# Khrylx/EgoPose

Measured on AMD Instinct MI355X. Metric: env-steps/sec (whole node) ego_mimic PPO, higher is better.
Workload: dtype f64 (rollout kernels K1-K6, physics state) + f32 (policy/value nets)

## Files before the change

egopose_amd/_lib.py:

```python
from __future__ import annotations

import ctypes as C
import os

HERE = os.path.dirname(os.path.abspath(__file__))
LIB_PATH = os.path.join(HERE, "libegopose_hip.so")

EGP_OK = 0
EGP_EXPERT_ROW = 168
EGP_LSTM_GATES_UNIT_MAJOR = 1

c_int_p = C.POINTER(C.c_int32)
c_dbl_p = C.POINTER(C.c_double)
vp = C.c_void_p


class ModelDesc(C.Structure):
    _fields_ = [
        ("nq", C.c_int32), ("nv", C.c_int32), ("nu", C.c_int32), ("nbody", C.c_int32), ("nM", C.c_int32),
        ("body_qpos_start", c_int_p), ("body_ndof", c_int_p), ("dof_parentid", c_int_p), ("dof_Madr", c_int_p),
        ("ee_body", c_int_p),
        ("jkp", c_dbl_p), ("jkd", c_dbl_p), ("a_ref", c_dbl_p), ("a_scale", c_dbl_p), ("torque_lim", c_dbl_p),
        ("b_diffw", c_dbl_p),
        ("sub_dt", C.c_double), ("frame_skip", C.c_int32), ("episode_len", C.c_int32),
# ... 37 lines not shown
class PolicyDesc(C.Structure):
    _fields_ = [("n", C.c_int32),
                ("ctx_rows", vp), ("ctx_row_stride", C.c_int64), ("ctx_dim", C.c_int32),
                ("t_idx", vp),
                ("state", vp), ("state_dim", C.c_int32),
                ("ctx", vp),
                ("qpos", vp), ("qvel", vp), ("phase_t", vp),
                ("zf_in", vp), ("zf_out", vp), ("clip", C.c_double),
                ("y", vp), ("y2", vp),
                ("zf_workspace", vp),
                ("layers", C.POINTER(MlpLayer)), ("n_layers", C.c_int32), ("activation", C.c_int32),
                ("log_std", vp), ("noise", vp),
                ("action", vp), ("mean_out", vp),
                ("cell", C.POINTER(MlpLayer)),
                ("h", vp), ("c", vp), ("hc_row_stride", C.c_int64),
                ("vctx_rows", vp), ("vctx_row_stride", C.c_int64), ("vctx_dim", C.c_int32),
                ("vlayers", C.POINTER(MlpLayer)), ("n_vlayers", C.c_int32), ("vactivation", C.c_int32),
                ("value_out", vp),
                ("stage_src", vp), ("stage_dst", vp), ("stage_bytes", C.c_int64)]


class LstmDesc(C.Structure):
    _fields_ = [("T", C.c_int32), ("B", C.c_int32), ("hidden", C.c_int32), ("n_problems", C.c_int32), ("reverse_mask", C.c_int32),
                ("w_hh", vp),
                ("gates_x", vp), ("ld_g", C.c_int32),
                ("h_out", vp * 4), ("ld_h", C.c_int32),
                ("gates_save", vp), ("cells_save", vp),
                ("last_only", C.c_int32),
                ("seq_base", vp),
                ("dh_out", vp * 4), ("ld_dh", C.c_int32),
                ("d_pre", vp),
                ("d_bias", vp), ("d_bias_rows", C.c_int32),
                ("seq_order", vp), ("seq_steps", vp), ("leave_skipped", C.c_int32)]


class GemmDesc(C.Structure):
    _fields_ = [("M", C.c_int32), ("N", C.c_int32), ("K", C.c_int32),
                ("A", vp), ("lda", C.c_int64), ("a_kcontig", C.c_int32),
                ("B", vp), ("ldb", C.c_int64), ("b_kcontig", C.c_int32),
                ("C", vp), ("ldc", C.c_int64),
                ("bias", vp), ("relu", C.c_int32),
                ("mask", vp), ("ldmask", C.c_int64),
                ("terms", C.c_int32), ("splits", C.c_int32), ("accumulate", C.c_int32),
                ("bias_grad", vp), ("workspace", vp),
                ("a_rows", vp), ("A2", vp), ("lda2", C.c_int64), ("a_split", C.c_int32), ("a_src_rows", C.c_int64),
                ("b_krows", vp), ("B2", vp), ("ldb2", C.c_int64), ("b_split", C.c_int32), ("b_src_rows", C.c_int64),
                ("c_rows", vp), ("a_krows", vp),
                ("act_kind", C.c_int32), ("mask_kind", C.c_int32)]


class PpoLossDesc(C.Structure):
    _fields_ = [("n", C.c_int32), ("n_pol", C.c_int32), ("act_dim", C.c_int32),
                ("rows", vp), ("pred", vp), ("returns", vp),
                ("mean", vp), ("ld_mean", C.c_int64),
                ("actions", vp), ("ld_act", C.c_int64),
                ("log_std", vp), ("adv", vp),
                ("fixed_logp", vp), ("write_fixed", C.c_int32),
                ("clip_eps", C.c_double), ("inv_n_val", C.c_double), ("inv_n_exp", C.c_double),
                ("d_pred", vp), ("d_mean", vp), ("ld_dmean", C.c_int64), ("d_log_std", vp),
                ("losses", vp), ("workspace", vp)]


class MinibatchPlanDesc(C.Structure):
    _fields_ = [("n", C.c_int32), ("state_dim", C.c_int32), ("act_dim", C.c_int32), ("batch", C.c_int32),
                ("perm", vp),
                ("states", vp), ("ld_states", C.c_int64),
# ... 142 lines not shown
    "egp_pose_features_f32": (C.c_int, [vp, vp, vp, vp, _i32, _i32, vp, vp, vp, vp, vp, vp, vp, vp]),
    "egp_zfilter_workspace_bytes": (_i64, [_i32, _i32]),
    "egp_zfilter_f64": (C.c_int, [vp, vp, _i32, _i32, vp, vp, _i32, _f64, vp, vp, vp]),
    "egp_zfilter_f32": (C.c_int, [vp, vp, _i32, _i32, vp, vp, _i32, _f64, vp, vp, vp]),
    "egp_obs_zfilter_f64": (C.c_int, [vp, vp, vp, vp, vp, _i32, vp, vp, _f64, vp, vp, _i32, vp, vp]),
    "egp_obs_zfilter_f32": (C.c_int, [vp, vp, vp, vp, vp, _i32, vp, vp, _f64, vp, vp, _i32, vp, vp]),
    "egp_gae_workspace_bytes": (_i64, [_i32]),
    "egp_gae_f64": (C.c_int, [vp, vp, vp, _i32, _f64, _f64, vp, vp, vp, vp, vp]),
    "egp_gae_f32": (C.c_int, [vp, vp, vp, _i32, _f64, _f64, vp, vp, vp, vp, vp]),
    "egp_gae_standardize_f64": (C.c_int, [vp, _i32, vp, vp]),
    "egp_gae_standardize_f32": (C.c_int, [vp, _i32, vp, vp]),
    "egp_lstm_gate_layout": (_i32, []),
    "egp_gather_concat_f32": (C.c_int, [vp, _i64, vp, vp, _i64, _i32, _i32, _i32, vp, _i64, vp]),
    "egp_scatter_rows_f32": (C.c_int, [vp, _i64, vp, _i32, _i32, vp, _i64, vp]),
    "egp_gemm_workspace_floats": (_i64, [_i32, _i32, _i32, _i32]),
    "egp_gemm_f32": (C.c_int, [C.POINTER(GemmDesc), vp]),
    "egp_ppo_loss_workspace_bytes": (_i64, [_i32, _i32, _i32]),
    "egp_ppo_loss_f32": (C.c_int, [C.POINTER(PpoLossDesc), vp]),
    "egp_ppo_stats_workspace_bytes": (_i64, [_i32, _i32, _i32]),
    "egp_ppo_stats_f32": (C.c_int, [C.POINTER(PpoStatsDesc), vp]),
    "egp_minibatch_plan_f32": (C.c_int, [C.POINTER(MinibatchPlanDesc), vp]),
    "egp_ppo_loss_mb_f32": (C.c_int, [C.POINTER(PpoLossMbDesc), vp]),
    "egp_gail_rows_f32": (C.c_int, [C.POINTER(GailRowsDesc), vp]),
    "egp_gail_rows_bwd_f32": (C.c_int, [C.POINTER(GailRowsDesc), vp]),
    "egp_bce_logits_workspace_bytes": (_i64, [_i32]),
    "egp_bce_logits_f32": (C.c_int, [C.POINTER(BceLogitsDesc), vp]),
    "egp_tcn_conv_f32": (C.c_int, [C.POINTER(TcnDesc), vp]),
    "egp_adam_workspace_bytes": (_i64, []),
    "egp_adam_step_f32": (C.c_int, [_i32, C.POINTER(AdamSegment), vp, vp, vp, vp, vp, vp, vp]),
    "egp_adam_step_f64": (C.c_int, [_i32, C.POINTER(AdamSegment), vp, vp, vp, vp, vp, vp, vp, vp]),
    "egp_adam_step_f64g": (C.c_int, [_i32, C.POINTER(AdamSegment), vp, vp, vp, vp, vp, vp, vp]),
    "egp_lstm_fwd_f32": (C.c_int, [C.POINTER(LstmDesc), vp]),
    "egp_lstm_bwd_f32": (C.c_int, [C.POINTER(LstmDesc), vp]),
    "egp_rollout_tick_pre": (C.c_int, [vp, _i32, _i32, _i32, _i32, vp, _i32, vp, vp]),
    "egp_rollout_tick_apply": (C.c_int, [vp, _i32, _i32, _i32, _i32, vp, vp]),
    "egp_obs_zfilter_split_max_rows": (C.c_int32, []),
    "egp_obs_zfilter_stats_f64": (C.c_int, [vp, vp, vp, vp, vp, _i32, vp, vp]),
    "egp_obs_zfilter_apply_f64": (C.c_int, [vp, vp, vp, vp, _i32, vp, vp, C.c_double, vp, vp, vp, vp]),
    "egp_rollout_tick_post": (C.c_int, [vp, _i32, _i32, _i32, _i32, vp, vp, vp, vp]),
    "egp_rollout_reset": (C.c_int, [vp, _i32, _i32, _i32, _i32, vp, _i32, vp, vp, vp, vp, vp, vp, vp, vp, vp]),
    "egp_engine_group_stream": (vp, [vp, _i32]),
    "egp_debug_burn": (C.c_int, [C.c_int64, _i32, vp, vp]),
    "egp_set_dynamics_model": (C.c_int, [vp, C.POINTER(DynamicsDesc)]),
    "egp_dynamics_f64": (C.c_int, [vp, vp, vp, _i32, vp, C.c_int64, vp, vp, vp]),
    "egp_set_pose2d_bodies": (C.c_int, [vp, c_int_p, c_int_p]),
    "egp_pose2d_f64": (C.c_int, [vp, vp, vp, vp, vp, vp, vp, C.c_int64, vp]),
    "egp_mlp_pack_floats": (C.c_int64, [_i32, _i32]),
    "egp_mlp_pack_f32": (C.c_int, [vp, C.c_int64, _i32, _i32, vp, vp]),
    "egp_policy_step_f32": (C.c_int, [C.POINTER(PolicyDesc), vp]),
    "egp_physics_register": (C.c_int, [C.POINTER(PhysicsVtable), _i32, C.POINTER(vp)]),
    "egp_physics_create_surrogate": (C.c_int, [C.POINTER(SurrogateDesc), _i32, C.POINTER(vp)]),
    "egp_physics_destroy": (C.c_int, [vp]),
    "egp_physics_name": (C.c_char_p, [vp]),
    "egp_physics_n_env": (_i32, [vp]),
    "egp_physics_reset_host": (C.c_int, [vp, _i32, vp, vp]),
    "egp_physics_step_host": (C.c_int, [vp, _i32, vp]),
    "egp_physics_drain_host": (C.c_int, [vp, _i32, vp, vp, vp, vp, vp]),
    "egp_engine_create": (C.c_int, [vp, vp, C.POINTER(EngineDesc), C.POINTER(vp)]),
    "egp_engine_destroy": (C.c_int, [vp]),
    "egp_engine_state": (C.c_int, [vp] + [C.POINTER(vp)] * 7),
    "egp_engine_reset": (C.c_int, [vp, vp, _i32, vp, vp, vp]),
    "egp_engine_step_async": (C.c_int, [vp, _i32, vp, vp, vp]),
    "egp_engine_wait": (C.c_int, [vp, _i32, vp]),
    "egp_engine_timing": (C.c_int, [vp, c_dbl_p, c_dbl_p, c_dbl_p, C.POINTER(_i64)]),
    "egp_engine_reset_timing": (C.c_int, [vp]),
    "egp_engine_inertia_uploads": (_i64, [vp]),
# ... 60 lines not shown
```

egopose_amd/csrc/egp_kernels.hip:

```cpp
#include <hip/hip_runtime.h>
#include <math.h>
#include <stdarg.h>
#include <stdio.h>
#include <stdlib.h>
#include <string.h>

#include <atomic>
#include <map>
#include <mutex>

#include "egp_internal.hpp"
#include "egp_dynamics_dev.hpp"
#include "egp_quat.hpp"
#include "egp_filter_dev.hpp"

namespace egp {

static thread_local char g_err[512] = "";
void set_error(const char *fmt, ...) {
    va_list ap;
    va_start(ap, fmt);
    vsnprintf(g_err, sizeof(g_err), fmt, ap);
    va_end(ap);
}
// ... 1713 lines not shown
static int dev_copy(egp_ctx *ctx, const T *host, size_t count, const T **out) {
    void *d = nullptr;
    EGP_HIP_CHECK(hipMalloc(&d, count * sizeof(T)));
    ctx->allocs.push_back(d);
    EGP_HIP_CHECK(hipMemcpy(d, host, count * sizeof(T), hipMemcpyHostToDevice));
    *out = (const T *)d;
    return EGP_OK;
}

static int fill_reward(egp_ctx *ctx, const egp_model_desc *d) {
    RewardW &w = ctx->rw;
    w.w_p = d->w_p; w.w_v = d->w_v; w.w_e = d->w_e; w.w_rp = d->w_rp; w.w_rv = d->w_rv;
    w.w_sum = d->w_p + d->w_v + d->w_e + d->w_rp + d->w_rv;
    w.k_p = d->k_p; w.k_v = d->k_v; w.k_e = d->k_e; w.k_rh = d->k_rh; w.k_rq = d->k_rq; w.k_rl = d->k_rl; w.k_ra = d->k_ra;
    w.v_ord = d->v_ord; w.decay = d->decay; w.episode_len = d->episode_len;
    EGP_REQUIRE(d->v_ord >= 1.0, "v_ord must be >= 1");
    EGP_REQUIRE(d->episode_len > 0, "episode_len must be positive");
    return EGP_OK;
}

extern "C" {

const char *egp_last_error(void) { return g_err; }
const char *egp_version(void) { return "egopose_hip 0.2.0 (gfx950)"; }
int64_t egp_abi_sizeof(const char *name) {
    if (!name) return -1;
#define EGP_ABI_SIZE(T) if (!strcmp(name, #T)) return (int64_t)sizeof(T);
    EGP_ABI_SIZE(egp_model_desc) EGP_ABI_SIZE(egp_expert_table) EGP_ABI_SIZE(egp_gemm_desc)
    EGP_ABI_SIZE(egp_dynamics_desc) EGP_ABI_SIZE(egp_mlp_layer) EGP_ABI_SIZE(egp_physics_vtable)
    EGP_ABI_SIZE(egp_surrogate_desc) EGP_ABI_SIZE(egp_engine_desc) EGP_ABI_SIZE(egp_rollout_tick)
    EGP_ABI_SIZE(egp_ppo_loss_desc) EGP_ABI_SIZE(egp_adam_segment) EGP_ABI_SIZE(egp_host_probe_result)
    EGP_ABI_SIZE(egp_minibatch_plan_desc) EGP_ABI_SIZE(egp_ppo_loss_mb_desc) EGP_ABI_SIZE(egp_tcn_desc)
    EGP_ABI_SIZE(egp_policy_desc) EGP_ABI_SIZE(egp_gail_rows_desc) EGP_ABI_SIZE(egp_bce_logits_desc)
    EGP_ABI_SIZE(egp_lstm_desc) EGP_ABI_SIZE(egp_ppo_stats_desc)
#undef EGP_ABI_SIZE
    return -1;
}
int32_t egp_obs_dim(const egp_ctx *ctx) { return ctx ? ctx->dm.obs_dim : -1; }

int egp_create(const egp_model_desc *d, int device, egp_ctx **out) {
    EGP_REQUIRE(d && out, "desc/out is NULL");
    EGP_REQUIRE(d->nv > 6 && d->nv <= EGP_MAX_NV, "nv must be in (6, 64]");
    EGP_REQUIRE(d->nq == d->nv + 1 && d->nu == d->nv - 6, "expects one free root joint + hinges (nq=nv+1, nu=nv-6)");
    EGP_REQUIRE(d->nbody >= 2 && d->nbody + 5 <= EGP_MAX_BODY, "nbody must be in [2, 27]");
    EGP_REQUIRE(d->nM > 0 && d->nM <= PD_NM_MAX, "nM out of range");
    EGP_REQUIRE(d->body_qpos_start && d->body_ndof && d->dof_parentid && d->dof_Madr && d->ee_body, "skeleton table is NULL");
    EGP_REQUIRE(d->jkp && d->jkd && d->a_ref && d->a_scale && d->torque_lim && d->b_diffw, "gain table is NULL");
    EGP_REQUIRE(d->sub_dt > 0 && d->frame_skip > 0, "timestep/frame_skip must be positive");
    EGP_REQUIRE(26 + 4 * (d->nbody - 1) <= 106 && 106 + 3 * (d->nbody - 1) <= EGP_EXPERT_ROW, "expert row overflow");
    EGP_HIP_CHECK(hipSetDevice(device));
    egp_ctx *ctx = new egp_ctx();
    ctx->device = device;
    ctx->frame_skip = d->frame_skip;
    int rc = fill_reward(ctx, d);
    if (rc != EGP_OK) { delete ctx; return rc; }
    DevModel &m = ctx->dm;
    m.nq = d->nq; m.nv = d->nv; m.nu = d->nu; m.nbody = d->nbody; m.nM = d->nM;
    m.sub_dt = d->sub_dt;
    m.dt = d->sub_dt * d->frame_skip;
    m.obs_heading = d->obs_heading != 0; m.obs_keep = d->obs_keep_root_heading != 0; m.obs_root = d->obs_coord_root != 0;
    m.obs_vel = d->obs_vel;
    m.action_torque = d->action_torque != 0;
    if (m.obs_vel < 0 || m.obs_vel > 2) { delete ctx; set_error("obs_vel must be 0 (full), 1 (root) or 2 (none)"); return EGP_E_INVALID; }
    m.obs_phase = d->obs_phase != 0;
    m.episode_len = d->episode_len;
    if (m.obs_phase && d->episode_len <= 0) { delete ctx; set_error("obs_phase needs episode_len > 0"); return EGP_E_INVALID; }
    m.obs_dim = obs_width(d->nq, d->nv, m.obs_heading, m.obs_vel, m.obs_phase);
// ... 592 lines not shown
```

egopose_amd/csrc/egp_lstm.hip:

```cpp
#include <hip/hip_runtime.h>
#include <math.h>
#include <stdlib.h>

#include "egp_internal.hpp"

namespace egp {

constexpr int KC = 64;

__device__ __forceinline__ float sigmoidf_(float x) { return __builtin_amdgcn_rcpf(1.0f + __expf(-x)); }
__device__ __forceinline__ float tanhf_(float x) { return 2.0f * __builtin_amdgcn_rcpf(1.0f + __expf(-2.0f * x)) - 1.0f; }

typedef float f32x4 __attribute__((ext_vector_type(4)));

template <typename V> __device__ __forceinline__ void st_save(V *p, V v) { __builtin_nontemporal_store(v, p); }
template <typename V> __device__ __forceinline__ V ld_save(const V *p) { return __builtin_nontemporal_load(p); }
template <typename V> __device__ __forceinline__ void st_dpre(V *p, V v) { __builtin_nontemporal_store(v, p); }

struct LstmGroup {
    int ld_g;
    int rev_mask;
    int ld_h;
    int ld_dh;
    long c_stride;
// ... 293 lines not shown
        for (int d = 0; d < PD; ++d) EGP_LSTM_FETCH(s0 - PD - d, d)
#pragma unroll
        for (int d = 0; d < PD; ++d)
            do_step(s0 - d, cg[d], cc_[d], cdh[d], d + 1 < PD ? cc_[d + 1 < PD ? d + 1 : 0] : pc[0]);
    }
#pragma unroll
    for (int d = 0; d < PD - 1; ++d)
        if (s0 - d >= 0) do_step(s0 - d, pg[d], pc[d], pdh[d], pc[d + 1]);
#undef EGP_LSTM_FETCH
    if (grp.db) {
        __syncthreads();
#pragma unroll
        for (int qq = 0; qq < NP; ++qq) {
            const int p = threadIdx.x + NT * qq;
            *reinterpret_cast<f32x4 *>(&s_d[p / LH][4 * (p % LH)]) = dsum[qq];
        }
        __syncthreads();
        if (grp.db_rows) {
            for (int p = threadIdx.x; p < ROWS * LG; p += NT) {
                const int r = p / LG, c = p % LG;
                if (FULL || r0 + r < B) grp.db[((long)prob * B + r0 + r) * LG + c] = s_d[r][c];
            }
        } else {
            for (int c = threadIdx.x; c < LG; c += NT) {
                float a = 0.f;
#pragma unroll
                for (int r = 0; r < ROWS; ++r) a += s_d[r][c];
                atomicAdd(grp.db + prob * LG + c, a);
            }
        }
    }
}

}

using namespace egp;

static int lstm_quads(int B) { return B >= 4096 ? 2 : 1; }

template <int NQ, int LH>
static void launch_fwd_mfma_t(bool full, bool train, bool last, int P, const float *gx, const float *w_hh, int T, int B, const LstmGroup &g,
                              float *gates_save, float *cells_save, hipStream_t s) {
    const dim3 grid((B + 4 * NQ - 1) / (4 * NQ), P), block(4 * LH);
    if (last && full) k_lstm_fwd_mfma<NQ, LH, true, LSTM_ST_LAST><<<grid, block, 0, s>>>(gx, w_hh, T, B, g, nullptr, nullptr);
    else if (last) k_lstm_fwd_mfma<NQ, LH, false, LSTM_ST_LAST><<<grid, block, 0, s>>>(gx, w_hh, T, B, g, nullptr, nullptr);
    else if (full && train) k_lstm_fwd_mfma<NQ, LH, true, LSTM_ST_TRAIN><<<grid, block, 0, s>>>(gx, w_hh, T, B, g, gates_save, cells_save);
    else if (full) k_lstm_fwd_mfma<NQ, LH, true, LSTM_ST_STEP><<<grid, block, 0, s>>>(gx, w_hh, T, B, g, gates_save, cells_save);
    else if (train) k_lstm_fwd_mfma<NQ, LH, false, LSTM_ST_TRAIN><<<grid, block, 0, s>>>(gx, w_hh, T, B, g, gates_save, cells_save);
    else k_lstm_fwd_mfma<NQ, LH, false, LSTM_ST_STEP><<<grid, block, 0, s>>>(gx, w_hh, T, B, g, gates_save, cells_save);
}
static void launch_fwd_mfma(int hidden, int P, const float *gx, const float *w_hh, int T, int B, const LstmGroup &g,
                            float *gates_save, float *cells_save, hipStream_t s, bool last = false) {
    const int nq = hidden == 64 ? lstm_quads(B) : 1;
    const bool full = B % (4 * nq) == 0, train = gates_save != nullptr;
    if (hidden == 128) launch_fwd_mfma_t<1, 128>(full, train, last, P, gx, w_hh, T, B, g, gates_save, cells_save, s);
    else if (nq >= 2) launch_fwd_mfma_t<2, 64>(full, train, last, P, gx, w_hh, T, B, g, gates_save, cells_save, s);
    else launch_fwd_mfma_t<1, 64>(full, train, last, P, gx, w_hh, T, B, g, gates_save, cells_save, s);
}

template <int NQ, int LH>
static void launch_bwd_mfma_t(bool full, int P, const float *gates_save, const float *cells_save, const float *w_hh, int T, int B,
                              const LstmGroup &g, float *d_pre, hipStream_t s) {
    const dim3 grid((B + 4 * NQ - 1) / (4 * NQ), P), block(4 * LH);
    if (full) k_lstm_bwd_mfma<NQ, LH, true><<<grid, block, 0, s>>>(gates_save, cells_save, w_hh, T, B, g, d_pre);
    else k_lstm_bwd_mfma<NQ, LH, false><<<grid, block, 0, s>>>(gates_save, cells_save, w_hh, T, B, g, d_pre);
}
// ... 22 lines not shown
    }
    const int ld_g = d->ld_g ? d->ld_g : 4 * H * P, ld_io = bwd ? d->ld_dh : d->ld_h;
    EGP_REQUIRE(ld_g >= 4 * H * P && ld_g % 4 == 0, "gate row stride below n_problems * 4H or not a multiple of 4");
    EGP_REQUIRE(ld_io == 0 || ld_io >= H, "h_out / dh_out row stride below the hidden size");
    EGP_REQUIRE((d->seq_order == nullptr) == (d->seq_steps == nullptr), "seq_order and seq_steps go together");
    EGP_REQUIRE((d->gates_save == nullptr) == (d->cells_save == nullptr), "gates_save and cells_save go together");
    EGP_REQUIRE(d->w_hh && (bwd ? d->gates_save && d->d_pre : d->gates_x != nullptr), "NULL pointer");
    if (!bwd) {
        EGP_REQUIRE(!d->seq_base || !d->gates_save || d->gates_save != d->gates_x,
                    "a frame table cannot double as the saved gates (rows are shared between sequences)");
        EGP_REQUIRE(!last || P == 1, "last_only sweeps one problem");
        EGP_REQUIRE(!last || !d->gates_save, "last_only saves nothing (inference)");
        EGP_REQUIRE(!last || !d->seq_order, "last_only takes no seq_order / seq_steps");
        EGP_REQUIRE(!last || d->seq_base, "last_only needs seq_base (windows of a frame table)");
    }
    LstmGroup g = {};
    g.ld_g = ld_g; g.rev_mask = d->reverse_mask; g.c_stride = (long)T * B * H;
    g.order = d->seq_order; g.steps = d->seq_steps; g.leave_skipped = d->seq_steps && d->leave_skipped;
    (bwd ? g.ld_dh : g.ld_h) = ld_io ? ld_io : H;
    for (int p = 0; p < P; ++p) {
        EGP_REQUIRE(bwd ? d->dh_out[p] != nullptr : d->h_out[p] != nullptr, "NULL h_out / dh_out of a problem");
        if (bwd) g.dh[p] = d->dh_out[p]; else g.h[p] = d->h_out[p];
    }
    if (bwd) {
        g.db = d->d_bias; g.db_rows = db_rows;
        launch_bwd_mfma(H, P, d->gates_save, d->cells_save, d->w_hh, T, B, g, d->d_pre, (hipStream_t)stream);
    } else {
        g.seq_base = d->seq_base;
        launch_fwd_mfma(H, P, d->gates_x, d->w_hh, T, B, g, d->gates_save, d->cells_save, (hipStream_t)stream, last);
    }
    return after_launch(bwd ? "k_lstm_bwd_mfma" : "k_lstm_fwd_mfma");
}

extern "C" {

int32_t egp_lstm_gate_layout(void) { return EGP_LSTM_GATES_UNIT_MAJOR; }
int egp_lstm_fwd_f32(const egp_lstm_desc *desc, void *stream) { return lstm_sweep(desc, false, stream); }
int egp_lstm_bwd_f32(const egp_lstm_desc *desc, void *stream) { return lstm_sweep(desc, true, stream); }

}
```

egopose_amd/lstm.py:

```python
from __future__ import annotations

import ctypes as C

import numpy as np
import torch

from . import _lib as L
from . import gemm as G

HIDDEN_SIZES = (64, 128)


def available(x, cell):
    return (x.is_cuda and x.dtype == torch.float32 and cell.hidden_size in HIDDEN_SIZES
            and cell.weight_hh.dtype == torch.float32 and cell.bias_ih is not None)


def _s():
    return L.current_stream()


_LAYOUT_CHECKED = False


# ... 69 lines not shown

    @staticmethod
    def backward(ctx, dh):
        lib = _lib()
        x2, w_in, w_hh, h_buf, gates, cells = ctx.saved_tensors
        T, B, D = ctx.shape
        HIDDEN = w_hh.shape[1]
        h = h_buf
        dpre = torch.empty(T, B, 4 * HIDDEN, dtype=h.dtype, device=h.device)
        dh = dh.contiguous()
        d = _desc(T, B, HIDDEN, 1, 1 if ctx.reverse else 0, w_hh, gates_save=gates, cells_save=cells,
                  dh_out=_slabs([dh.data_ptr()]), d_pre=dpre)
        L.check(lib.egp_lstm_bwd_f32(d, _s()), "egp_lstm_bwd_f32")
        h_prev = h_buf[1:] if ctx.reverse else h_buf[:T]
        _, inv = _gate_perm(HIDDEN, h.device)
        if G.enabled():
            d2 = dpre.view(T * B, 4 * HIDDEN)
            dw_ih, dbias = G.linear_wgrad(d2, x2, want_bias=True)
            dw_hh = G.linear_wgrad(d2, h_prev.reshape(T * B, HIDDEN), want_bias=False)
            dw_ih, dw_hh, dbias = dw_ih.index_select(0, inv), dw_hh.index_select(0, inv), dbias.index_select(0, inv)
            d_w_ih = dw_ih if ctx.needs_input_grad[1] else None
            d_w_hh = dw_hh if ctx.needs_input_grad[2] else None
            d_b = dbias if (ctx.needs_input_grad[3] or ctx.needs_input_grad[4]) else None
        else:
            xh1 = torch.cat((x2.view(T, B, D), h_prev, h.new_ones(T, B, 1)), 2)
            dw = torch.bmm(dpre.transpose(1, 2), xh1).sum(0).index_select(0, inv)
            d_w_ih = dw[:, :D].contiguous() if ctx.needs_input_grad[1] else None
            d_w_hh = dw[:, D:D + HIDDEN].contiguous() if ctx.needs_input_grad[2] else None
            d_b = dw[:, D + HIDDEN].contiguous() if (ctx.needs_input_grad[3] or ctx.needs_input_grad[4]) else None
        d_x = dpre.view(T * B, 4 * HIDDEN).mm(w_in).view(T, B, D) if ctx.needs_input_grad[0] else None
        return d_x, d_w_ih, d_w_hh, d_b, d_b, None, None


class LstmGroup(torch.autograd.Function):

    @staticmethod
    def forward(ctx, x, reverse_mask, P, width, train, ragged, frames, *params):
        lib = _lib()
        T, B, D = x.shape
        w_ih, w_hh, b_ih, b_hh = params[0::4], params[1::4], params[2::4], params[3::4]
        H = w_hh[0].shape[1]
        x2 = x.reshape(T * B, D)
        pord = [p for p in range(P) if not (reverse_mask >> p) & 1] + [p for p in range(P) if (reverse_mask >> p) & 1]
        nf = sum(1 for p in range(P) if not (reverse_mask >> p) & 1)
        kmask = sum(1 << q for q in range(nf, P))
        bperm, _ = _stacked_perm(H, P, x.device)
        w_in = torch.cat([w_ih[p] for p in pord], 0).index_select(0, bperm)
        bias = (torch.cat([b_ih[p] for p in pord]) + torch.cat([b_hh[p] for p in pord])).index_select(0, bperm)
        rows = None
        if ragged is not None and ragged.rows is not None and 0 < nf and G.enabled() and G.fused_rows_available() \
                and ragged.T == T and ragged.rows.shape[0] >= 4096 and D >= 32:
            rows = ragged.rows
        seq_base, gates_buf = None, None
        if frames is not None and G.enabled():
            table, seq_base = frames
            gx = G.linear_fwd(table, w_in, bias)
            gates_buf = torch.empty(T * B, P * 4 * H, dtype=x.dtype, device=x.device) if train else None
        elif rows is not None:
            gx = torch.empty(T * B, P * 4 * H, dtype=x.dtype, device=x.device)
            nfc = nf * 4 * H
            G.gemm(x2, w_in[:nfc], True, True, bias=bias[:nfc], a_rows=rows, c_rows=rows, out=gx[:, :nfc])
            if nf < P:
                G.gemm(x2, w_in[nfc:], True, True, bias=bias[nfc:], out=gx[:, nfc:])
        elif G.enabled():
            gx = G.linear_fwd(x2, w_in, bias)
        else:
            gx = torch.addmm(bias, x2, w_in.t())
        w_hh_all = torch.stack([w_hh[p].contiguous() for p in pord], 0)
        n_out, W = P // width, width * H
        h_buf = torch.empty(n_out, T + 2, B, W, dtype=x.dtype, device=x.device)
        h_buf[:, 0].zero_()
        h_buf[:, T + 1].zero_()
        cells = torch.empty(P, T, B, H, dtype=x.dtype, device=x.device) if train else None
        base, esz = h_buf.data_ptr(), h_buf.element_size()
        ptrs = _slabs([base + esz * (((p // width) * (T + 2) + 1) * B * W + (p % width) * H) for p in pord])
        order, steps = (ragged.order, ragged.steps) if ragged is not None else (None, None)
        leave = int(rows is not None and train)
        gates = gates_buf if seq_base is not None else (gx if train else None)
        d = _desc(T, B, H, P, kmask, w_hh_all, gates_x=gx, h_out=ptrs, ld_h=W, gates_save=gates, cells_save=cells, seq_base=seq_base,
                  seq_order=order, seq_steps=steps, leave_skipped=leave)
        L.check(lib.egp_lstm_fwd_f32(d, _s()), "egp_lstm_fwd_f32")
        outs = tuple(h_buf[i, 1:T + 1] for i in range(n_out))
        if train:
            ctx.save_for_backward(x2, w_in, w_hh_all, h_buf, gates, cells)
            ctx.meta = (T, B, D, H, P, width, reverse_mask)
            ctx.ragged, ctx.rows, ctx.pord, ctx.nf, ctx.kmask, ctx.leave = ragged, rows, pord, nf, kmask, leave
        return outs

    @staticmethod
    def backward(ctx, *douts):
        lib = _lib()
        x2, w_in, w_hh_all, h_buf, gates, cells = ctx.saved_tensors
        T, B, D, H, P, width, reverse_mask = ctx.meta
        W = width * H
        _, inv = _gate_perm(H, x2.device)
        douts = [d.contiguous() if d is not None else h_buf.new_zeros(T, B, W) for d in douts]
        ragged, rows, pord, nf, kmask = ctx.ragged, ctx.rows, ctx.pord, ctx.nf, ctx.kmask
        esz = h_buf.element_size()
        ptrs = _slabs([douts[p // width].data_ptr() + esz * (p % width) * H for p in pord])
        dpre = torch.empty(T * B, P * 4 * H, dtype=x2.dtype, device=x2.device)
        db_rows = torch.empty(P, B, 4 * H, dtype=x2.dtype, device=x2.device)
        order, steps = (ragged.order, ragged.steps) if ragged is not None else (None, None)
        leave = int(bool(ctx.leave) and not ctx.needs_input_grad[0])
        d = _desc(T, B, H, P, kmask, w_hh_all, gates_save=gates, cells_save=cells, dh_out=ptrs, ld_dh=W, d_pre=dpre,
                  d_bias=db_rows, d_bias_rows=1, seq_order=order, seq_steps=steps, leave_skipped=leave)
        L.check(lib.egp_lstm_bwd_f32(d, _s()), "egp_lstm_bwd_f32")
        db = db_rows.sum(1)
        d3 = dpre.view(T, B, P * 4 * H)
        use_g = G.enabled()
        nfc = nf * 4 * H
        if rows is not None:
            n_rows = rows.shape[0]
            parts = [G.gemm(dpre[:, :nfc], x2, False, False, splits=G.pick_splits(nfc, D, n_rows), a_krows=rows, b_krows=rows)]
            if nf < P:
                parts.append(G.linear_wgrad(dpre[:, nfc:], x2, want_bias=False))
            dw_ih_all = torch.cat(parts, 0)
        elif use_g:
            dw_ih_all = G.linear_wgrad(dpre, x2, want_bias=False)
        else:
            dw_ih_all = torch.bmm(d3.transpose(1, 2), x2.view(T, B, D)).sum(0)
        grads = [None] * (4 * P)
        _, binv = _stacked_perm(H, P, x2.device)
        dw_ih_t = dw_ih_all.index_select(0, binv)
        db_t = db.reshape(-1).index_select(0, binv).view(P, 4 * H)
        for q, p in enumerate(pord):
            rev = (kmask >> q) & 1
            slab = h_buf[p // width, 2:] if rev else h_buf[p // width, :T]
            h_prev = slab[:, :, (p % width) * H:(p % width + 1) * H]
            if use_g:
                dq, hq = dpre[:, q * 4 * H:(q + 1) * 4 * H], slab.reshape(T * B, W)[:, (p % width) * H:(p % width + 1) * H]
                if rows is not None and not rev:
                    dw_hh = G.gemm(dq, hq, False, False, splits=G.pick_splits(4 * H, H, rows.shape[0]), a_krows=rows, b_krows=rows).index_select(0, inv)
                else:
                    dw_hh = G.linear_wgrad(dq, hq, want_bias=False).index_select(0, inv)
            else:
                dw_hh = torch.bmm(d3[:, :, q * 4 * H:(q + 1) * 4 * H].transpose(1, 2), h_prev).sum(0).index_select(0, inv)
            dw_ih = dw_ih_t[q * 4 * H:(q + 1) * 4 * H]
            d_b = db_t[q]
            grads[4 * p:4 * p + 4] = [dw_ih, dw_hh, d_b, d_b]
        d_x = dpre.mm(w_in).view(T, B, D) if ctx.needs_input_grad[0] else None
        return (d_x, None, None, None, None, None, None, *grads)


def _wants_grad(x, params):
    return torch.is_grad_enabled() and (x.requires_grad or any(p.requires_grad for p in params))


def group_available(x, cells):
    if not cells or len(cells) > 4:
        return False
    c0 = cells[0]
    return all(available(x, c) and c.hidden_size == c0.hidden_size and c.input_size == c0.input_size for c in cells)


class Ragged:

    def __init__(self, order, steps, rows, n_seq, T):
        self.order, self.steps, self.rows, self.n_seq, self.T = order, steps, rows, n_seq, T


def ragged_order(seq_steps, device, T=None):
    st = np.asarray(torch.as_tensor(seq_steps).cpu().numpy(), dtype=np.int64).reshape(-1)
    B = st.shape[0]
    order = np.argsort(-st, kind="stable")
    st_sorted = st[order]
    rows = None
    if T is not None and B > 0:
        wg = np.maximum.reduceat(st_sorted, np.arange(0, B, 8))
        t_wg = np.minimum(np.repeat(wg, 8)[:B], int(T))
        n = int(t_wg.sum())
        if n < 0.9 * T * B:
            t_seq = np.empty(B, np.int64)
            t_seq[order] = t_wg
            stepped = np.arange(int(T), dtype=np.int64)[:, None] < t_seq[None, :]
            rows = torch.as_tensor(np.flatnonzero(stepped), dtype=torch.int64, device=device)
    return Ragged(torch.as_tensor(order, dtype=torch.int32, device=device), torch.as_tensor(st_sorted, dtype=torch.int32, device=device),
                  rows, B, T)


def lstm_group(x, cells, reverses, pairs=False, ragged=None, frames=None):
    mask = sum(1 << i for i, r in enumerate(reverses) if r)
    params = [t for c in cells for t in (c.weight_ih, c.weight_hh, c.bias_ih, c.bias_hh)]
    if ragged is not None and ragged.n_seq != x.shape[1]:
        ragged = None
    if frames is not None:
        table, base = frames
        ok = (table.is_cuda and table.dtype == x.dtype and table.dim() == 2 and table.shape[1] == x.shape[2] and table.is_contiguous()
              and base.dtype == torch.int32 and base.is_cuda and base.is_contiguous() and base.shape[0] == x.shape[1] and not x.requires_grad)
        if not ok:
            frames = None
    return list(LstmGroup.apply(x.contiguous(), mask, len(cells), 2 if pairs else 1, _wants_grad(x, params), ragged, frames, *params))


WINDOW_CALLS = 0


def window_available(table, cell):
    return available(table, cell)


@torch.no_grad()
def window_last(cell, table, seq_base, steps, reverse, out):
    global WINDOW_CALLS
    H, B = cell.hidden_size, seq_base.shape[0]
    if not (table.dim() == 2 and table.is_contiguous() and window_available(table, cell)):
        raise ValueError("window_last needs a contiguous float32 (F, D) table on the device and an LSTMCell of hidden size 64 or 128")
    if not (seq_base.is_cuda and seq_base.dtype == torch.int32 and seq_base.dim() == 1 and seq_base.is_contiguous()):
        raise ValueError("seq_base must be a contiguous int32 device vector")
    if not (out.is_cuda and out.dtype == torch.float32 and out.shape == (B, H) and (H == 1 or out.stride(1) == 1)
            and (B <= 1 or out.stride(0) >= H)):
        raise ValueError("out must be float32 (B, H) = (%d, %d) device rows, got %s" % (B, H, tuple(out.shape)))
    if steps < 1:
        raise ValueError("a window has at least one step, got %d" % steps)
    if B == 0:
        return out
    lo, hi = int(seq_base.min()), int(seq_base.max())
    if lo < 0 or hi + steps > table.shape[0]:
        raise ValueError("windows [%d, %d) leave the table's %d frames" % (lo, hi + steps, table.shape[0]))
    perm, _ = _gate_perm(H, table.device)
    w_in, bias = cell.weight_ih.index_select(0, perm), (cell.bias_ih + cell.bias_hh).index_select(0, perm)
    gx = G.linear_fwd(table, w_in.contiguous(), bias) if G.enabled() else torch.addmm(bias, table, w_in.t())
    w_hh = cell.weight_hh.contiguous()
    d = _desc(int(steps), B, H, 1, 1 if reverse else 0, w_hh, gates_x=gx, h_out=_slabs([out.data_ptr()]),
              ld_h=out.stride(0) if B > 1 else max(out.stride(0), H), last_only=1, seq_base=seq_base)
# ... 9 lines not shown
```

egopose_amd/nets.py:

```python
from __future__ import annotations

import collections
import math
import os

import numpy as np
import torch
import torch.nn as nn

from . import dist as _dist
from . import gemm as _gemm
from . import gemm_tuning as _tuning
from . import lstm as _hip_lstm
from . import tcn as _tcn
from .tcn import TemporalConvNet

_LSTM_IMPL = os.environ.get("EGP_LSTM", "hip")

_ACT = {"tanh": torch.tanh, "relu": torch.relu, "sigmoid": torch.sigmoid}


def bucket_rows(x):
    if _tuning.enabled() and x.is_cuda and x.dim() == 2 and x.shape[0] >= 4 * _tuning.ROW_BUCKET:
        pad = _tuning.pad_to(x.shape[0], _tuning.ROW_BUCKET)
# ... 351 lines not shown
    def __init__(self, cnn_feat_dim, v_hdim=128, v_margin=10, v_net_type="lstm", v_net_param=None, causal=False):
        super().__init__()
        self.cnn_feat_dim, self.v_hdim, self.v_margin, self.v_net_type = cnn_feat_dim, v_hdim, v_margin, v_net_type
        self.v_net = _video_net(cnn_feat_dim, v_hdim, v_net_type, v_net_param, causal)
        self._gather_tm = None
        self._gather_unique = False
        self._ragged = None
        self._frames = None
        self._v_ctx = None

    def _extent(self, length):
        return self.v_margin, length + self.v_margin

    def initialize(self, x):
        m = self.v_margin
        if self.mode == "test":
            x = self._to_params(x)
            single = x.dim() == 2
            out = self.forward_v_net(x.unsqueeze(1) if single else x)[m:-m]
            self.v_out = out.squeeze(1) if single else out
            self.t = 0
            return
        masks, cnn_feat, v_metas = x
        device, dtype = masks.device, masks.dtype
        self._frames = None
        ep = _segment_episodes(masks, v_metas)
        self.indices = idx = ep.indices
        max_len = ep.max_len
        meta = self._train_windows(ep, cnn_feat, device, dtype, max_len)
        table = self._table_on(device)
        n_rows = self.cnn_feat_ctx.shape[0] * self.cnn_feat_ctx.shape[1]
        if table is not None and table.dtype == dtype and table.is_contiguous() and 2 * table.shape[0] <= n_rows:
            base = self._take_offset_host[meta[:, 0].astype(np.int64)] + meta[:, 1].astype(np.int64) - m
            self._frames = (table, torch.as_tensor(base.astype(np.int32), device=device))
        self.gather_indices = torch.as_tensor(idx, dtype=torch.long, device=device)
        tm = ((idx % max_len) + m) * self.cnn_feat_ctx.shape[1] + idx // max_len
        self._gather_tm = torch.as_tensor(tm, dtype=torch.long, device=device)
        self._gather_unique = ep.covered == masks.shape[0] or np.unique(tm).size == tm.size
        steps = np.zeros(self.cnn_feat_ctx.shape[1], np.int64)
        steps[:len(ep.lens)] = ep.lens + m
        lstm_ctx = self.cnn_feat_ctx.is_cuda and isinstance(self.v_net, RNN)
        self._ragged = _hip_lstm.ragged_order(steps, device, T=self.cnn_feat_ctx.shape[0]) if lstm_ctx else None

    @torch.no_grad()
    def online_contexts(self, x):
        if self.mode != "test":
            raise RuntimeError("online_contexts is a test-mode (evaluation) call")
        m = self.v_margin
        x = self._to_params(x)
        if x.dim() != 2 or x.shape[0] < 2 * m + 1:
            raise ValueError("online_contexts takes one take's features (T + 2m, D) with T >= 1, got %s" % (tuple(x.shape),))
        T, net = x.shape[0] - 2 * m, self.v_net
        offline = lambda: self.forward_v_net(x.unsqueeze(1))[m:m + T, 0]
        if isinstance(net, _tcn.TemporalConvNet):
            reach = (net.kernel_size - 1) * (2 ** len(net.network) - 1)
            if net.causal or reach <= m:
                return offline()
            return torch.stack([self.forward_v_net(x[:t + 2 * m + 1].unsqueeze(1))[t + m, 0] for t in range(T)], 0)
        if not net.bi_dir:
            return offline()
        H = net.rnn_f.hidden_size
        out = x.new_empty(T, 2 * H)
        out[:, :H] = net._sweep(net.rnn_f, x.unsqueeze(1), False)[m:m + T, 0]
        if net.cell_type == "lstm" and _LSTM_IMPL != "torch" and _hip_lstm.window_available(x, net.rnn_b):
            base = torch.arange(m, m + T, dtype=torch.int32, device=x.device)
            _hip_lstm.window_last(net.rnn_b, x.contiguous(), base, m + 1, True, out[:, H:])
        else:
# ... 330 lines not shown
```

include/egopose_hip.h:

```cpp
#ifndef EGOPOSE_HIP_H
#define EGOPOSE_HIP_H

#include <stdint.h>

#ifdef __cplusplus
extern "C" {
#endif

#define EGP_OK 0
#define EGP_E_INVALID (-1)
#define EGP_E_HIP (-2)
#define EGP_E_STATE (-3)
#define EGP_E_PHYSICS (-4)

#define EGP_MAX_NV 64
#define EGP_MAX_BODY 32
#define EGP_EXPERT_ROW 168

typedef struct egp_ctx egp_ctx;
typedef struct egp_physics egp_physics;
typedef struct egp_engine egp_engine;

typedef struct egp_model_desc {
    int32_t nq, nv, nu, nbody, nM;
// ... 266 lines not shown

struct egp_tcn_desc {
    int32_t T, B, C_in, C_out, taps, shift0, dshift;
    const float *X; int64_t ldx;
    const float *W;
    const float *bias; int32_t relu;
    const float *mask; int64_t ldmask;
    const float *gate; int64_t ldgate;
    const float *X2; int64_t ldx2; int32_t C2; const float *W2; const float *b2; int32_t x2_after_act;
    float *out; int64_t ldout;
    float *out2; int64_t ldout2;
};
typedef struct egp_tcn_desc egp_tcn_desc;
int egp_tcn_conv_f32(const egp_tcn_desc *desc, void *stream);

#define EGP_LSTM_GATES_TORCH 0
#define EGP_LSTM_GATES_UNIT_MAJOR 1
int32_t egp_lstm_gate_layout(void);
typedef struct egp_lstm_desc {
    int32_t T, B, hidden, n_problems, reverse_mask;
    const float *w_hh;
    const float *gates_x; int32_t ld_g;
    float *h_out[4]; int32_t ld_h;
    float *gates_save; float *cells_save;
    int32_t last_only;
    const int32_t *seq_base;
    const float *dh_out[4]; int32_t ld_dh;
    float *d_pre;
    float *d_bias; int32_t d_bias_rows;
    const int32_t *seq_order; const int32_t *seq_steps; int32_t leave_skipped;
} egp_lstm_desc;
int egp_lstm_fwd_f32(const egp_lstm_desc *desc, void *stream);
int egp_lstm_bwd_f32(const egp_lstm_desc *desc, void *stream);

typedef struct egp_dynamics_desc {
    int32_t nbody, njoint;
    const int32_t *body_parent;
    const double *body_pos;
    const double *body_com;
    const double *body_inertia;
    const double *body_mass;
    const int32_t *body_ndof;
    const double *joint_axis;
    const double *joint_anchor;
    double armature;
    double gravity[3];
} egp_dynamics_desc;
int egp_set_dynamics_model(egp_ctx *ctx, const egp_dynamics_desc *desc);
int egp_dynamics_f64(egp_ctx *ctx, const double *qpos, const double *qvel, int32_t n, double *qM, int64_t ld_m,
                     double *qfrc_bias, double *xpos, void *stream);

#define EGP_POSE2D_NKP 12
int egp_set_pose2d_bodies(egp_ctx *ctx, const int32_t *kp_body , const int32_t *roles );
int egp_pose2d_f64(egp_ctx *ctx, const double *qpos , const double *gt ,
                   const int32_t *flip , double *p_out , double *dist ,
                   int32_t *valid , int64_t n, void *stream);


typedef struct egp_mlp_layer {
    const float *wt;
    const float *bias;
    int32_t in_dim, out_dim;
} egp_mlp_layer;
int64_t egp_mlp_pack_floats(int32_t in_dim, int32_t out_dim);
int egp_mlp_pack_f32(const float *weight, int64_t ldw, int32_t in_dim, int32_t out_dim, float *packed, void *stream);
typedef struct egp_policy_desc {
// ... 128 lines not shown
```

Before: 981,000.

## Compute LSTM input-weight gradient via per-frame summed d_pre against shared frame table

When LSTM inputs are overlapping windows into a shared frame table and no input gradient is needed, the backward pass first sums d_pre over all window rows that map to each table frame with a new gather kernel. It then runs a single weight-gradient GEMM of the per-frame sums against the much smaller table, and the bias gradient comes from the same GEMM. This replaces a GEMM over all T*B window rows and the per-row bias buffer. It adds a host-built frame index (argsort/searchsorted), a new ragged fwd_len tensor, and a gather kernel whose work depends on how many windows overlap each frame.

```diff
diff --git a/egopose_amd/_lib.py b/egopose_amd/_lib.py
--- a/egopose_amd/_lib.py
+++ b/egopose_amd/_lib.py
@@ -93,6 +93,14 @@
                 ("d_pre", vp),
                 ("d_bias", vp), ("d_bias_rows", C.c_int32),
                 ("seq_order", vp), ("seq_steps", vp), ("leave_skipped", C.c_int32)]
+
+
+class LstmFrameSumDesc(C.Structure):
+    _fields_ = [("T", C.c_int32), ("B", C.c_int32), ("F", C.c_int32),
+                ("d_pre", vp), ("ld_g", C.c_int32),
+                ("seq_base", vp), ("by_base", vp), ("first", vp),
+                ("fwd_len", vp), ("n_fwd_cols", C.c_int32),
+                ("S", vp)]
 
 
 class GemmDesc(C.Structure):
@@ -301,6 +309,7 @@
     "egp_adam_step_f64g": (C.c_int, [_i32, C.POINTER(AdamSegment), vp, vp, vp, vp, vp, vp, vp]),
     "egp_lstm_fwd_f32": (C.c_int, [C.POINTER(LstmDesc), vp]),
     "egp_lstm_bwd_f32": (C.c_int, [C.POINTER(LstmDesc), vp]),
+    "egp_lstm_frame_sum_f32": (C.c_int, [C.POINTER(LstmFrameSumDesc), vp]),
     "egp_rollout_tick_pre": (C.c_int, [vp, _i32, _i32, _i32, _i32, vp, _i32, vp, vp]),
     "egp_rollout_tick_apply": (C.c_int, [vp, _i32, _i32, _i32, _i32, vp, vp]),
     "egp_obs_zfilter_split_max_rows": (C.c_int32, []),
diff --git a/egopose_amd/csrc/egp_kernels.hip b/egopose_amd/csrc/egp_kernels.hip
--- a/egopose_amd/csrc/egp_kernels.hip
+++ b/egopose_amd/csrc/egp_kernels.hip
@@ -1769,7 +1769,7 @@
     EGP_ABI_SIZE(egp_ppo_loss_desc) EGP_ABI_SIZE(egp_adam_segment) EGP_ABI_SIZE(egp_host_probe_result)
     EGP_ABI_SIZE(egp_minibatch_plan_desc) EGP_ABI_SIZE(egp_ppo_loss_mb_desc) EGP_ABI_SIZE(egp_tcn_desc)
     EGP_ABI_SIZE(egp_policy_desc) EGP_ABI_SIZE(egp_gail_rows_desc) EGP_ABI_SIZE(egp_bce_logits_desc)
-    EGP_ABI_SIZE(egp_lstm_desc) EGP_ABI_SIZE(egp_ppo_stats_desc)
+    EGP_ABI_SIZE(egp_lstm_desc) EGP_ABI_SIZE(egp_ppo_stats_desc) EGP_ABI_SIZE(egp_lstm_frame_sum_desc)
 #undef EGP_ABI_SIZE
     return -1;
 }
diff --git a/egopose_amd/csrc/egp_lstm.hip b/egopose_amd/csrc/egp_lstm.hip
--- a/egopose_amd/csrc/egp_lstm.hip
+++ b/egopose_amd/csrc/egp_lstm.hip
@@ -349,6 +349,38 @@
     }
 }
 
+template <int U>
+__global__ __launch_bounds__(512) void k_lstm_frame_sum(const float *__restrict__ dpre, int ld, int T, int B, const int *__restrict__ seq_base,
+                                                        const int *__restrict__ by_base, const int *__restrict__ first,
+                                                        const int *__restrict__ fwd_len, int n_fwd_cols, float *__restrict__ S) {
+    const int f = blockIdx.x, c = 4 * threadIdx.x;
+    const bool ragged_col = fwd_len != nullptr && c < n_fwd_cols;
+    const int *__restrict__ len_of = fwd_len ? fwd_len : seq_base;
+    const int j0 = max(first[max(f - T + 1, 0)], 0), j1 = min(first[f + 1], B);
+    f32x4 acc = f32x4{0.f, 0.f, 0.f, 0.f};
+    for (int j = j0; j < j1; j += U) {
+        int b[U], t[U], len[U];
+#pragma unroll
+        for (int i = 0; i < U; ++i) b[i] = by_base[min(j + i, j1 - 1)];
+#pragma unroll
+        for (int i = 0; i < U; ++i) {
+            const int bb = (unsigned)b[i] < (unsigned)B ? b[i] : 0;
+            t[i] = f - seq_base[bb];
+            len[i] = len_of[bb];
+        }
+        f32x4 v[U];
+#pragma unroll
+        for (int i = 0; i < U; ++i) {
+            v[i] = f32x4{0.f, 0.f, 0.f, 0.f};
+            if (j + i < j1 && (unsigned)b[i] < (unsigned)B && (unsigned)t[i] < (unsigned)T && (!ragged_col || t[i] < len[i]))
+                v[i] = ld_save(reinterpret_cast<const f32x4 *>(dpre + ((long)t[i] * B + b[i]) * ld + c));
+        }
+#pragma unroll
+        for (int i = 0; i < U; ++i) acc += v[i];
+    }
+    *reinterpret_cast<f32x4 *>(S + (long)f * ld + c) = acc;
+}
+
 }
 
 using namespace egp;
@@ -437,8 +469,27 @@
     return after_launch(bwd ? "k_lstm_bwd_mfma" : "k_lstm_fwd_mfma");
 }
 
+static int lstm_frame_sum(const egp_lstm_frame_sum_desc *d, void *stream) {
+    EGP_REQUIRE(d, "desc is NULL");
+    const int T = d->T, B = d->B, F = d->F, ld = d->ld_g;
+    EGP_REQUIRE(T >= 0 && B >= 0 && F >= 0, "negative size");
+    if (F == 0) return EGP_OK;
+    EGP_REQUIRE(ld >= 4 && ld % 4 == 0 && ld <= 2048, "ld_g must be a multiple of 4 in 4..2048");
+    EGP_REQUIRE(d->n_fwd_cols >= 0 && d->n_fwd_cols <= ld && d->n_fwd_cols % 4 == 0, "n_fwd_cols must be a multiple of 4 in 0..ld_g");
+    EGP_REQUIRE(d->S, "NULL pointer");
+    if (T == 0 || B == 0) {
+        EGP_HIP_CHECK(hipMemsetAsync(d->S, 0, sizeof(float) * (size_t)F * ld, (hipStream_t)stream));
+        return EGP_OK;
+    }
+    EGP_REQUIRE(d->d_pre && d->seq_base && d->by_base && d->first, "NULL pointer");
+    k_lstm_frame_sum<8><<<dim3(F), dim3(ld / 4), 0, (hipStream_t)stream>>>(d->d_pre, ld, T, B, d->seq_base, d->by_base, d->first, d->fwd_len,
+                                                                          d->n_fwd_cols, d->S);
+    return after_launch("k_lstm_frame_sum");
+}
+
 extern "C" {
 
+int egp_lstm_frame_sum_f32(const egp_lstm_frame_sum_desc *desc, void *stream) { return lstm_frame_sum(desc, stream); }
 int32_t egp_lstm_gate_layout(void) { return EGP_LSTM_GATES_UNIT_MAJOR; }
 int egp_lstm_fwd_f32(const egp_lstm_desc *desc, void *stream) { return lstm_sweep(desc, false, stream); }
 int egp_lstm_bwd_f32(const egp_lstm_desc *desc, void *stream) { return lstm_sweep(desc, true, stream); }
diff --git a/egopose_amd/lstm.py b/egopose_amd/lstm.py
--- a/egopose_amd/lstm.py
+++ b/egopose_amd/lstm.py
@@ -125,6 +125,9 @@
         return d_x, d_w_ih, d_w_hh, d_b, d_b, None, None
 
 
+D_PRE_TAP = None
+
+
 class LstmGroup(torch.autograd.Function):
 
     @staticmethod
@@ -144,9 +147,9 @@
         if ragged is not None and ragged.rows is not None and 0 < nf and G.enabled() and G.fused_rows_available() \
                 and ragged.T == T and ragged.rows.shape[0] >= 4096 and D >= 32:
             rows = ragged.rows
-        seq_base, gates_buf = None, None
+        seq_base, gates_buf, findex = None, None, None
         if frames is not None and G.enabled():
-            table, seq_base = frames
+            table, seq_base, findex = frames
             gx = G.linear_fwd(table, w_in, bias)
             gates_buf = torch.empty(T * B, P * 4 * H, dtype=x.dtype, device=x.device) if train else None
         elif rows is not None:
@@ -178,6 +181,7 @@
             ctx.save_for_backward(x2, w_in, w_hh_all, h_buf, gates, cells)
             ctx.meta = (T, B, D, H, P, width, reverse_mask)
             ctx.ragged, ctx.rows, ctx.pord, ctx.nf, ctx.kmask, ctx.leave = ragged, rows, pord, nf, kmask, leave
+            ctx.frames = (table, seq_base, findex) if findex is not None else None
         return outs
 
     @staticmethod
@@ -192,17 +196,26 @@
         esz = h_buf.element_size()
         ptrs = _slabs([douts[p // width].data_ptr() + esz * (p % width) * H for p in pord])
         dpre = torch.empty(T * B, P * 4 * H, dtype=x2.dtype, device=x2.device)
-        db_rows = torch.empty(P, B, 4 * H, dtype=x2.dtype, device=x2.device)
+        by_frame = ctx.frames is not None and not ctx.needs_input_grad[0]
+        db_rows = None if by_frame else torch.empty(P, B, 4 * H, dtype=x2.dtype, device=x2.device)
         order, steps = (ragged.order, ragged.steps) if ragged is not None else (None, None)
         leave = int(bool(ctx.leave) and not ctx.needs_input_grad[0])
         d = _desc(T, B, H, P, kmask, w_hh_all, gates_save=gates, cells_save=cells, dh_out=ptrs, ld_dh=W, d_pre=dpre,
-                  d_bias=db_rows, d_bias_rows=1, seq_order=order, seq_steps=steps, leave_skipped=leave)
+                  d_bias=db_rows, d_bias_rows=0 if by_frame else 1, seq_order=order, seq_steps=steps, leave_skipped=leave)
         L.check(lib.egp_lstm_bwd_f32(d, _s()), "egp_lstm_bwd_f32")
-        db = db_rows.sum(1)
+        if D_PRE_TAP is not None:
+            D_PRE_TAP.append(dpre)
         d3 = dpre.view(T, B, P * 4 * H)
         use_g = G.enabled()
         nfc = nf * 4 * H
-        if rows is not None:
+        if by_frame:
+            table, seq_base, findex = ctx.frames
+            fwd_len = ragged.fwd_len if ragged is not None and ragged.T == T else None
+            if leave and fwd_len is None:
+                raise L.EgpError("LstmGroup: a ragged batch with unwritten d_pre rows needs Ragged.fwd_len (ragged_order(..., T=T))")
+            S = frame_sum(dpre, T, B, seq_base, findex, fwd_len, nfc)
+            dw_ih_all, db = G.linear_wgrad(S, table, want_bias=True)
+        elif rows is not None:
             n_rows = rows.shape[0]
             parts = [G.gemm(dpre[:, :nfc], x2, False, False, splits=G.pick_splits(nfc, D, n_rows), a_krows=rows, b_krows=rows)]
             if nf < P:
@@ -212,6 +225,8 @@
             dw_ih_all = G.linear_wgrad(dpre, x2, want_bias=False)
         else:
             dw_ih_all = torch.bmm(d3.transpose(1, 2), x2.view(T, B, D)).sum(0)
+        if not by_frame:
+            db = db_rows.sum(1)
         grads = [None] * (4 * P)
         _, binv = _stacked_perm(H, P, x2.device)
         dw_ih_t = dw_ih_all.index_select(0, binv)
@@ -248,8 +263,8 @@
 
 class Ragged:
 
-    def __init__(self, order, steps, rows, n_seq, T):
-        self.order, self.steps, self.rows, self.n_seq, self.T = order, steps, rows, n_seq, T
+    def __init__(self, order, steps, rows, n_seq, T, fwd_len=None):
+        self.order, self.steps, self.rows, self.n_seq, self.T, self.fwd_len = order, steps, rows, n_seq, T, fwd_len
 
 
 def ragged_order(seq_steps, device, T=None):
@@ -257,32 +272,72 @@
     B = st.shape[0]
     order = np.argsort(-st, kind="stable")
     st_sorted = st[order]
-    rows = None
+    rows = fwd_len = None
     if T is not None and B > 0:
         wg = np.maximum.reduceat(st_sorted, np.arange(0, B, 8))
         t_wg = np.minimum(np.repeat(wg, 8)[:B], int(T))
         n = int(t_wg.sum())
+        t_seq = np.empty(B, np.int64)
+        t_seq[order] = t_wg
+        fwd_len = torch.as_tensor(t_seq.astype(np.int32), device=device)
         if n < 0.9 * T * B:
-            t_seq = np.empty(B, np.int64)
-            t_seq[order] = t_wg
             stepped = np.arange(int(T), dtype=np.int64)[:, None] < t_seq[None, :]
             rows = torch.as_tensor(np.flatnonzero(stepped), dtype=torch.int64, device=device)
     return Ragged(torch.as_tensor(order, dtype=torch.int32, device=device), torch.as_tensor(st_sorted, dtype=torch.int32, device=device),
-                  rows, B, T)
-
-
-def lstm_group(x, cells, reverses, pairs=False, ragged=None, frames=None):
+                  rows, B, T, fwd_len)
+
+
+class FrameIndex:
+
+    def __init__(self, by_base, first, n_seq, T, F):
+        self.by_base, self.first, self.n_seq, self.T, self.F = by_base, first, n_seq, T, F
+
+
+def frame_index(base, T, F, device):
+    bs = np.asarray(torch.as_tensor(base).cpu().numpy(), dtype=np.int64).reshape(-1)
+    if bs.size and (bs.min() < 0 or bs.max() + int(T) > int(F)):
+        raise ValueError("windows [%d, %d) leave the table's %d frames" % (bs.min(), bs.max() + int(T), F))
+    by = np.argsort(bs, kind="stable")
+    first = np.searchsorted(bs[by], np.arange(int(F) + 1), side="left")
+    return FrameIndex(torch.as_tensor(by.astype(np.int32), device=device), torch.as_tensor(first.astype(np.int32), device=device),
+                      bs.size, int(T), int(F))
+
+
+def frame_sum(d_pre, T, B, seq_base, index, fwd_len=None, n_fwd_cols=0, out=None):
+    ld = d_pre.shape[1]
+    ok = (d_pre.is_cuda and d_pre.dtype == torch.float32 and d_pre.dim() == 2 and d_pre.is_contiguous() and d_pre.shape[0] == T * B
+          and index.n_seq == B and index.T == T and seq_base.is_cuda and seq_base.dtype == torch.int32 and seq_base.is_contiguous()
+          and seq_base.shape[0] == B
+          and (fwd_len is None or (fwd_len.is_cuda and fwd_len.dtype == torch.int32 and fwd_len.is_contiguous() and fwd_len.shape[0] == B))
+          and (out is None or (out.is_cuda and out.dtype == torch.float32 and out.shape == (index.F, ld) and out.is_contiguous())))
+    if not ok:
+        raise ValueError("frame_sum: d_pre must be contiguous float32 (T*B, ld) rows, the index and the int32 lists those of its %d windows" % B)
+    S = out if out is not None else torch.empty(index.F, ld, dtype=torch.float32, device=d_pre.device)
+    d = L.LstmFrameSumDesc(T=T, B=B, F=index.F, d_pre=d_pre.data_ptr(), ld_g=ld, seq_base=seq_base.data_ptr(),
+                           by_base=index.by_base.data_ptr(), first=index.first.data_ptr(),
+                           fwd_len=fwd_len.data_ptr() if fwd_len is not None else None, n_fwd_cols=n_fwd_cols, S=S.data_ptr())
+    L.check(_lib().egp_lstm_frame_sum_f32(d, _s()), "egp_lstm_frame_sum_f32")
+    return S
+
+
+def lstm_group(x, cells, reverses, pairs=False, ragged=None, frames=None, frame_wgrad=True):
     mask = sum(1 << i for i, r in enumerate(reverses) if r)
     params = [t for c in cells for t in (c.weight_ih, c.weight_hh, c.bias_ih, c.bias_hh)]
+    train = _wants_grad(x, params)
     if ragged is not None and ragged.n_seq != x.shape[1]:
         ragged = None
     if frames is not None:
-        table, base = frames
+        table, base = frames[0], frames[1]
         ok = (table.is_cuda and table.dtype == x.dtype and table.dim() == 2 and table.shape[1] == x.shape[2] and table.is_contiguous()
               and base.dtype == torch.int32 and base.is_cuda and base.is_contiguous() and base.shape[0] == x.shape[1] and not x.requires_grad)
-        if not ok:
-            frames = None
-    return list(LstmGroup.apply(x.contiguous(), mask, len(cells), 2 if pairs else 1, _wants_grad(x, params), ragged, frames, *params))
+        index = None
+        if ok and frame_wgrad and train and G.enabled():
+            T, B, F = x.shape[0], x.shape[1], table.shape[0]
+            index = frames[2] if len(frames) > 2 else None
+            if index is None or (index.n_seq, index.T, index.F) != (B, T, F):
+                index = frame_index(base, T, F, x.device)
+        frames = (table, base, index) if ok else None
+    return list(LstmGroup.apply(x.contiguous(), mask, len(cells), 2 if pairs else 1, train, ragged, frames, *params))
 
 
 WINDOW_CALLS = 0
diff --git a/egopose_amd/nets.py b/egopose_amd/nets.py
--- a/egopose_amd/nets.py
+++ b/egopose_amd/nets.py
@@ -407,7 +407,10 @@
         n_rows = self.cnn_feat_ctx.shape[0] * self.cnn_feat_ctx.shape[1]
         if table is not None and table.dtype == dtype and table.is_contiguous() and 2 * table.shape[0] <= n_rows:
             base = self._take_offset_host[meta[:, 0].astype(np.int64)] + meta[:, 1].astype(np.int64) - m
-            self._frames = (table, torch.as_tensor(base.astype(np.int32), device=device))
+            findex = None
+            if table.is_cuda and isinstance(self.v_net, RNN):
+                findex = _hip_lstm.frame_index(base, self.cnn_feat_ctx.shape[0], table.shape[0], device)
+            self._frames = (table, torch.as_tensor(base.astype(np.int32), device=device), findex)
         self.gather_indices = torch.as_tensor(idx, dtype=torch.long, device=device)
         tm = ((idx % max_len) + m) * self.cnn_feat_ctx.shape[1] + idx // max_len
         self._gather_tm = torch.as_tensor(tm, dtype=torch.long, device=device)
diff --git a/include/egopose_hip.h b/include/egopose_hip.h
--- a/include/egopose_hip.h
+++ b/include/egopose_hip.h
@@ -322,6 +322,16 @@
 } egp_lstm_desc;
 int egp_lstm_fwd_f32(const egp_lstm_desc *desc, void *stream);
 int egp_lstm_bwd_f32(const egp_lstm_desc *desc, void *stream);
+
+struct egp_lstm_frame_sum_desc {
+    int32_t T, B, F;
+    const float *d_pre; int32_t ld_g;
+    const int32_t *seq_base; const int32_t *by_base; const int32_t *first;
+    const int32_t *fwd_len; int32_t n_fwd_cols;
+    float *S;
+};
+typedef struct egp_lstm_frame_sum_desc egp_lstm_frame_sum_desc;
+int egp_lstm_frame_sum_f32(const egp_lstm_frame_sum_desc *desc, void *stream);
 
 typedef struct egp_dynamics_desc {
     int32_t nbody, njoint;
```

Result: slower. 947,100 (-3.5%).
